# slitvinov/PINN_for_quantum_wavefunction_surfaces

Measured on NVIDIA B200. Metric: collocation points/sec per training step (fwd+lap+bwd), higher is better.
Workload: dtype f32

## Files before the change

### include/pinn_b200.h

```cpp
#ifndef PINN_B200_H
#define PINN_B200_H

#include <stdint.h>

#ifdef __cplusplus
extern "C" {
#endif

#define PINN_THETA_SIZE 1521
#define PINN_NUM_TENSORS 16
#define PINN_SUMS_SIZE 8

#define PINN_VARIANT_POC 0
#define PINN_VARIANT_TRAINPY 1

#define PINN_F32 0
#define PINN_F64 1

#define PINN_EINVAL (-1)
#define PINN_ENOTSUP (-2)
#define PINN_ETIMEDOUT (-3)

typedef struct pinn_handle pinn_handle;

int pinn_version(void);
int pinn_theta_size(void);
void pinn_theta_offsets(int* out);

int pinn_create(int device, pinn_handle** out);
int pinn_destroy(pinn_handle* h);
const char* pinn_last_error(pinn_handle* h);
int64_t pinn_launch_count(pinn_handle* h);

#define PINN_ENGINE_FFMA 0
#define PINN_ENGINE_TCGEN05 1
int pinn_set_engine(pinn_handle* h, int engine);
int pinn_get_engine(pinn_handle* h);

int pinn_measure_fp32_peak(pinn_handle* h, double* fma_per_s, double* ms, double* sm_mhz);
int pinn_step_kernel_clock(pinn_handle* h, void* stream, double* cycles, double* ns);

int pinn_host_timing(pinn_handle* h, double* out4);

int pinn_profile_begin(pinn_handle* h);
int pinn_profile_collect(pinn_handle* h, double* total_ms, int* launches);

int pinn_loss_fwd_bwd(pinn_handle* h, int variant, int64_t n,
                      const void* x, const void* y, const void* z, const void* R, int in_dtype,
                      const uint8_t* mask, const float* theta, const double* weights,
                      uint32_t grad_mask, float bcutoff,
                      double* sums, double* dtheta, float* E_out, void* stream);

int pinn_fields(pinn_handle* h, int variant, int64_t n,
                const void* x, const void* y, const void* z, const void* R, int in_dtype,
                const float* theta,
                float* psi, float* lap, float* hpsi, float* res, float* E, void* stream);

int pinn_loss_fwd_bwd_tensors(pinn_handle* h, int variant, int64_t n,
                              const void* x, const void* y, const void* z, const void* R, int in_dtype,
                              const uint8_t* mask, const void* const* params, int param_dtype, int param_layout,
                              const double* weights_host, uint32_t grad_mask, float bcutoff,
                              double* sums, double* dtheta, void* E_out, int E_dtype, void* stream);

int pinn_mask_from_index_sets(pinn_handle* h, int64_t n, const int64_t* idx1, int64_t n1, const int64_t* idx2, int64_t n2,
                              uint8_t* mask, void* stream);

int pinn_loss_fwd_bwd_host(pinn_handle* h, int variant, int64_t n,
                           const void* x, const void* y, const void* z, const void* R, int in_dtype,
                           const uint8_t* mask, const double* theta_host, const double* weights_host,
                           uint32_t grad_mask, float bcutoff,
// ... 61 lines not shown
```

### pinn_for_quantum_wavefunction_surfaces_b200/_lib.py

```python
import ctypes
import os
import threading

_HERE = os.path.dirname(os.path.abspath(__file__))
_LIB_NAME = "libpinn_b200.so"

EXPORTS = [
    "pinn_version", "pinn_theta_size", "pinn_theta_offsets", "pinn_create", "pinn_destroy", "pinn_last_error",
    "pinn_launch_count", "pinn_set_engine", "pinn_get_engine", "pinn_profile_begin", "pinn_profile_collect", "pinn_loss_fwd_bwd", "pinn_fields", "pinn_loss_fwd_bwd_host",
    "pinn_loss_fwd_bwd_tensors", "pinn_mask_from_index_sets", "pinn_measure_fp32_peak", "pinn_step_kernel_clock",
    "pinn_sample", "pinn_adam_step", "pinn_enet_curve", "pinn_grid_reduce", "pinn_spheroidal_reduce", "pinn_trainer_create", "pinn_trainer_destroy",
    "pinn_trainer_load_state", "pinn_trainer_set_batch", "pinn_trainer_run", "pinn_trainer_read", "pinn_trainer_batch",
    "pinn_trainer_stream",
    "pinn_host_timing", "pinn_dp_init", "pinn_dp_connect", "pinn_dp_connect_local", "pinn_dp_enable", "pinn_dp_status", "pinn_dp_set_timeout", "pinn_dp_shutdown",
]


class TrainConfig(ctypes.Structure):
    _fields_ = [("variant", ctypes.c_int), ("best_mode", ctypes.c_int), ("history_mean_E", ctypes.c_int),
                ("sc_sampling", ctypes.c_int), ("n", ctypes.c_int64), ("freeze_after", ctypes.c_int64),
                ("best_after", ctypes.c_int64), ("history_capacity", ctypes.c_int64), ("seed", ctypes.c_uint64),
                ("xL", ctypes.c_float), ("xR", ctypes.c_float), ("yL", ctypes.c_float), ("yR", ctypes.c_float),
                ("zL", ctypes.c_float), ("zR", ctypes.c_float), ("RL", ctypes.c_float), ("RR", ctypes.c_float),
                ("cutoff", ctypes.c_float), ("bcutoff", ctypes.c_float), ("grad_mask", ctypes.c_uint32),
                ("lr", ctypes.c_double), ("beta1", ctypes.c_double), ("beta2", ctypes.c_double), ("eps", ctypes.c_double)]


class PinnError(RuntimeError):
    pass


def library_path():
    return os.environ.get("PINN_B200_LIBRARY") or os.path.join(_HERE, _LIB_NAME)


_lib = None
_lock = threading.Lock()


def lib():
    global _lib
    with _lock:
        if _lib is not None:
            return _lib
        path = library_path()
        if not os.path.exists(path):
            raise PinnError("%s not found: build it with `python -c 'import __graft_entry__ as g; g.build()'` "
                            "(there is no CPU fallback)" % path)
        L = ctypes.CDLL(path)
        vp, i32, i64, u32, f32 = ctypes.c_void_p, ctypes.c_int, ctypes.c_int64, ctypes.c_uint32, ctypes.c_float
        L.pinn_version.restype = i32
        L.pinn_theta_size.restype = i32
        L.pinn_theta_offsets.argtypes = [ctypes.POINTER(i32)]
        L.pinn_theta_offsets.restype = None
        L.pinn_create.argtypes = [i32, ctypes.POINTER(vp)]
        L.pinn_create.restype = i32
        L.pinn_destroy.argtypes = [vp]
        L.pinn_destroy.restype = i32
        L.pinn_last_error.argtypes = [vp]
        L.pinn_last_error.restype = ctypes.c_char_p
        L.pinn_launch_count.argtypes = [vp]
        L.pinn_launch_count.restype = i64
        L.pinn_set_engine.argtypes = [vp, i32]
        L.pinn_set_engine.restype = i32
        L.pinn_get_engine.argtypes = [vp]
        L.pinn_get_engine.restype = i32
        L.pinn_profile_begin.argtypes = [vp]
        L.pinn_profile_begin.restype = i32
        L.pinn_profile_collect.argtypes = [vp, ctypes.POINTER(ctypes.c_double), ctypes.POINTER(i32)]
        L.pinn_profile_collect.restype = i32
        L.pinn_loss_fwd_bwd.argtypes = [vp, i32, i64, vp, vp, vp, vp, i32, vp, vp, vp, u32, f32, vp, vp, vp, vp]
        L.pinn_loss_fwd_bwd.restype = i32
        L.pinn_loss_fwd_bwd_tensors.argtypes = [vp, i32, i64, vp, vp, vp, vp, i32, vp, vp, i32, i32, vp, u32, f32, vp, vp, vp, i32, vp]
        L.pinn_loss_fwd_bwd_tensors.restype = i32
        L.pinn_mask_from_index_sets.argtypes = [vp, i64, vp, i64, vp, i64, vp, vp]
        L.pinn_mask_from_index_sets.restype = i32
        L.pinn_measure_fp32_peak.argtypes = [vp, ctypes.POINTER(ctypes.c_double), ctypes.POINTER(ctypes.c_double),
                                             ctypes.POINTER(ctypes.c_double)]
        L.pinn_measure_fp32_peak.restype = i32
        L.pinn_step_kernel_clock.argtypes = [vp, vp, ctypes.POINTER(ctypes.c_double), ctypes.POINTER(ctypes.c_double)]
        L.pinn_step_kernel_clock.restype = i32
        L.pinn_fields.argtypes = [vp, i32, i64, vp, vp, vp, vp, i32, vp, vp, vp, vp, vp, vp, vp]
        L.pinn_fields.restype = i32
        L.pinn_loss_fwd_bwd_host.argtypes = [vp, i32, i64, vp, vp, vp, vp, i32, vp, vp, vp, u32, f32, vp, vp, vp]
        L.pinn_loss_fwd_bwd_host.restype = i32
        u64, f64 = ctypes.c_uint64, ctypes.c_double
        L.pinn_sample.argtypes = [vp, i64, u64, u64, ctypes.POINTER(f32), f32, f32, vp, vp, vp, vp, vp, vp, vp, vp]
        L.pinn_sample.restype = i32
        L.pinn_adam_step.argtypes = [vp, vp, vp, vp, vp, vp, vp, vp, vp, vp, vp, vp, i64, i64, f64, f64, f64, f64, u32,
                                     i32, i64, i32, vp]
        L.pinn_adam_step.restype = i32
        L.pinn_enet_curve.argtypes = [vp, vp, vp, i32, vp, vp, vp, vp, vp]
        L.pinn_enet_curve.restype = i32
        L.pinn_grid_reduce.argtypes = [vp, i32, vp, i32, i32, i32, ctypes.POINTER(f64), f64, vp, vp, vp, vp, vp]
        L.pinn_grid_reduce.restype = i32
        L.pinn_spheroidal_reduce.argtypes = [vp, i32, vp, i32, vp, i32, vp, vp, i32, vp, vp, vp, vp]
        L.pinn_spheroidal_reduce.restype = i32
        L.pinn_trainer_create.argtypes = [vp, ctypes.POINTER(TrainConfig), vp, ctypes.POINTER(vp)]
        L.pinn_trainer_create.restype = i32
# ... 60 lines not shown
    _cache = {}
    _cache_lock = threading.Lock()

    def __init__(self, device=0):
        self.L = lib()
        self.device = int(device)
        hp = ctypes.c_void_p()
        rc = self.L.pinn_create(self.device, ctypes.byref(hp))
        if rc != 0:
            raise PinnError("pinn_create(device=%d) failed (%d): %s"
                            % (device, rc, self.L.pinn_last_error(None).decode()))
        self.h = hp

    @classmethod
    def get(cls, device=0):
        device = int(device)
        with cls._cache_lock:
            if device not in cls._cache:
                cls._cache[device] = Handle(device)
            return cls._cache[device]

    def check(self, rc, what):
        if rc != 0:
            raise PinnError("%s failed (%d): %s" % (what, rc, self.L.pinn_last_error(self.h).decode()))

    def launch_count(self):
        return int(self.L.pinn_launch_count(self.h))

    ENGINES = {"ffma": 0, "tcgen05": 1}

    def set_engine(self, name):
        self.check(self.L.pinn_set_engine(self.h, self.ENGINES[name]), "pinn_set_engine")

    def get_engine(self):
        return {v: k for k, v in self.ENGINES.items()}[int(self.L.pinn_get_engine(self.h))]

    def measure_fp32_peak(self):
        r, ms, mhz = ctypes.c_double(), ctypes.c_double(), ctypes.c_double()
        self.check(self.L.pinn_measure_fp32_peak(self.h, ctypes.byref(r), ctypes.byref(ms), ctypes.byref(mhz)), "pinn_measure_fp32_peak")
        return 2.0 * r.value, ms.value, mhz.value

    def step_kernel_clock(self, stream):
        c, ns = ctypes.c_double(), ctypes.c_double()
        self.check(self.L.pinn_step_kernel_clock(self.h, ctypes.c_void_p(stream), ctypes.byref(c), ctypes.byref(ns)), "pinn_step_kernel_clock")
        return c.value / ns.value * 1e3 if ns.value > 0 else 0.0

    def profile_begin(self):
        self.check(self.L.pinn_profile_begin(self.h), "pinn_profile_begin")

    def profile_collect(self):
        ms, k = ctypes.c_double(), ctypes.c_int()
        self.check(self.L.pinn_profile_collect(self.h, ctypes.byref(ms), ctypes.byref(k)), "pinn_profile_collect")
        return ms.value, k.value

    DP_HANDLE_BYTES = 64

    def dp_init(self, rank, world, want_ipc=True):
        buf = ctypes.create_string_buffer(self.DP_HANDLE_BYTES)
        self.check(self.L.pinn_dp_init(self.h, int(rank), int(world), buf if want_ipc else None), "pinn_dp_init")
        return bytes(buf.raw)

    def dp_connect(self, all_handles):
        blob = b"".join(all_handles)
        self.check(self.L.pinn_dp_connect(self.h, ctypes.c_char_p(blob)), "pinn_dp_connect")

    def dp_connect_local(self, handles):
# ... 27 lines not shown
```

### pinn_for_quantum_wavefunction_surfaces_b200/csrc/pinn_capi.cu

```cuda
#include <chrono>
#include <cstdio>
#include <cstdlib>
#include <cstring>
#include <mutex>
#include <string>
#include <vector>

#include "pinn_handle.h"
#include "pinn_train.h"

std::string g_create_err;

constexpr int HOST_IN_THETA = 1536;
constexpr size_t HOST_IN_BYTES = HOST_IN_THETA * sizeof(float) + 4 * sizeof(double);

static const int kOffsets[17] = {O_W1, O_B1, O_W2, O_B2, O_WO, O_BO, O_WE1, O_BE1, O_WE2, O_BE2, O_WE, O_BE,
                                 O_WGL, O_BGL, O_WG, O_BG, NTHETA};

extern "C" {

int pinn_version(void) { return 100; }
int pinn_theta_size(void) { return NTHETA; }
void pinn_theta_offsets(int* out) { memcpy(out, kOffsets, sizeof(kOffsets)); }

// ... 24 lines not shown
#ifdef PINN_AB_BUILD
  if (const char* e = getenv("PINN_B200_ENGINE")) {
    if (!strcmp(e, "ffma")) h->engine = PINN_ENGINE_FFMA;
    else if (!strcmp(e, "tcgen05")) h->engine = PINN_ENGINE_TCGEN05;
  }
  if (const char* e = getenv("PINN_B200_HOST_ZEROCOPY")) h->host_zero_copy = strcmp(e, "0") != 0;
  if (const char* e = getenv("PINN_B200_HOST_INLINE")) h->host_inline_params = strcmp(e, "0") != 0;
  CREATE_CU(cudaMalloc(&h->wts, sizeof(Wts)));
#endif
  CREATE_CU(cudaMalloc(&h->theta_dev, HOST_IN_BYTES));
  h->weights_dev = reinterpret_cast<double*>(h->theta_dev + HOST_IN_THETA);
  CREATE_CU(cudaHostAlloc(&h->out_pinned, NPART * sizeof(double), cudaHostAllocMapped));
  CREATE_CU(cudaHostGetDevicePointer(&h->out_mapped, h->out_pinned, 0));
  CREATE_CU(cudaMallocHost(&h->theta_pinned, HOST_IN_BYTES));
  h->weights_pinned = reinterpret_cast<double*>(h->theta_pinned + HOST_IN_THETA);
  CREATE_CU(cudaStreamCreateWithFlags(&h->s_copy, cudaStreamNonBlocking));
  CREATE_CU(cudaStreamCreateWithFlags(&h->s_main, cudaStreamNonBlocking));
  CREATE_CU(cudaEventCreateWithFlags(&h->ev_copy, cudaEventDisableTiming));
  for (int c = 0; c < 4; c++) CREATE_CU(cudaEventCreateWithFlags(&h->ev_chunk[c], cudaEventDisableTiming));
  if (!ws_for(h, h->s_main, 4 * h->sm_count)) {
    const std::string msg = h->err;
    pinn_destroy(h);
    g_create_err = "pinn_create: " + msg;
    return PINN_EINVAL;
  }
  *out = h;
  return 0;
}

}

static void ws_free(pinn_workspace& w) {
  cudaFree(w.partials); cudaFree(w.weights); cudaFree(w.counts); cudaFree(w.grid_partials); cudaFree(w.sph_partials);
  w = pinn_workspace();
}

void ws_release(pinn_handle* h, cudaStream_t st) {
  for (pinn_workspace& c : h->ws)
    if (c.stream == st && c.partials) {
      cudaStreamSynchronize(st);
      ws_free(c);
    }
}

static bool stream_is_capturing(cudaStream_t st) {
  cudaStreamCaptureStatus cap = cudaStreamCaptureStatusNone;
  if (cudaStreamIsCapturing(st, &cap) != cudaSuccess) { cudaGetLastError(); return false; }
  return cap != cudaStreamCaptureStatusNone;
}

pinn_workspace* ws_for(pinn_handle* h, cudaStream_t st, int rows) {
  constexpr size_t MAX_WS = 32;
  pinn_workspace* w = nullptr;
  for (pinn_workspace& c : h->ws)
    if (c.stream == st && c.partials) { w = &c; break; }
  if (w && w->rows >= rows) {
    if (!w->in_graph && stream_is_capturing(st)) w->in_graph = true;
    w->last_use = ++h->ws_clock;
    return w;
  }
  if (stream_is_capturing(st)) {
    fail(h, PINN_EINVAL, "first call on a stream under CUDA-graph capture: call once on this stream outside the capture first");
    return nullptr;
  }
  if (!w) {
    for (pinn_workspace& c : h->ws)
      if (!c.partials) { w = &c; break; }
    if (!w && h->ws.size() >= MAX_WS) {
      size_t lru = h->ws.size();
      for (size_t i = 0; i < h->ws.size(); i++)
        if (!h->ws[i].in_graph && h->ws[i].stream != h->s_main && (lru == h->ws.size() || h->ws[i].last_use < h->ws[lru].last_use)) lru = i;
      if (lru == h->ws.size()) {
        fail(h, PINN_EINVAL, "more than 32 streams with captured graphs or trainers on one handle");
        return nullptr;
      }
      cudaDeviceSynchronize();
      ws_free(h->ws[lru]);
      w = &h->ws[lru];
    } else if (!w) {
      h->ws.emplace_back();
      w = &h->ws.back();
    }
  } else {
    if (w->in_graph) {
      fail(h, PINN_EINVAL, "this stream's workspace is referenced by a captured graph and cannot grow");
      return nullptr;
    }
    cudaStreamSynchronize(st);
    ws_free(*w);
  }
  w->stream = st;
  cudaError_t e = cudaMalloc(&w->partials, (size_t)rows * NPART * sizeof(double));
  if (e == cudaSuccess) e = cudaMalloc(&w->weights, 4 * sizeof(double));
  if (e == cudaSuccess) e = cudaMalloc(&w->counts, 4 * sizeof(unsigned long long));
  if (e == cudaSuccess) e = cudaMemset(w->counts, 0, 4 * sizeof(unsigned long long));
  if (e == cudaSuccess) e = cudaMalloc(&w->grid_partials, (size_t)(h->sm_count + 1) * 8 * sizeof(double));
  if (e != cudaSuccess) {
    ws_free(*w);
    fail(h, (int)e, "workspace allocation (cudaMalloc)");
    return nullptr;
  }
  w->rows = rows;
  w->last_use = ++h->ws_clock;
  return w;
}

bool ws_sph_rows(pinn_handle* h, pinn_workspace* w, cudaStream_t st, int rows) {
  if (w->sph_rows >= rows) return true;
  if (stream_is_capturing(st)) {
    fail(h, PINN_EINVAL, "spheroidal sweep larger than any earlier one on a stream under CUDA-graph capture: make the largest "
                         "call once on this stream outside the capture first");
    return false;
  }
  if (w->in_graph) {
    fail(h, PINN_EINVAL, "this stream's workspace is referenced by a captured graph and cannot grow");
    return false;
  }
  cudaStreamSynchronize(st);
  cudaFree(w->sph_partials);
  w->sph_partials = nullptr;
  w->sph_rows = 0;
  cudaError_t e = cudaMalloc(&w->sph_partials, (size_t)rows * 8 * sizeof(double));
  if (e != cudaSuccess) {
    w->sph_partials = nullptr;
    fail(h, (int)e, "spheroidal workspace allocation (cudaMalloc)");
    return false;
  }
  w->sph_rows = rows;
  return true;
// ... 33 lines not shown
  DevGuard dev_guard(h->device);
  dp_release(h);
  cudaDeviceSynchronize();
#ifdef PINN_AB_BUILD
  cudaFree(h->wts);
#endif
  for (pinn_workspace& w : h->ws) ws_free(w);
  cudaFree(h->theta_dev); cudaFree(h->stage_dev);
  cudaFreeHost(h->out_pinned); cudaFreeHost(h->theta_pinned);
  if (h->s_copy) cudaStreamDestroy(h->s_copy);
  if (h->s_main) cudaStreamDestroy(h->s_main);
  if (h->ev_copy) cudaEventDestroy(h->ev_copy);
  for (int c = 0; c < 4; c++) if (h->ev_chunk[c]) cudaEventDestroy(h->ev_chunk[c]);
  for (cudaEvent_t e : h->ev_pool) cudaEventDestroy(e);
  delete h;
  return 0;
}

const char* pinn_last_error(pinn_handle* h) { return h ? h->err.c_str() : g_create_err.c_str(); }
int64_t pinn_launch_count(pinn_handle* h) { return h ? h->launches : 0; }

int pinn_set_engine(pinn_handle* h, int engine) {
  if (!h) return PINN_EINVAL;
  std::lock_guard<std::mutex> lk(h->mu);
  if (engine != PINN_ENGINE_FFMA && engine != PINN_ENGINE_TCGEN05) return fail(h, PINN_EINVAL, "pinn_set_engine: unknown engine");
#ifndef PINN_AB_BUILD
  if (engine != PINN_ENGINE_TCGEN05)
    return fail(h, PINN_ENOTSUP, "pinn_set_engine: this library carries the tcgen05 engine only (the FFMA engine exists in A/B builds, tools/build_ab.sh)");
#endif
  h->engine = engine;
  return 0;
}
int pinn_get_engine(pinn_handle* h) { return h ? h->engine : PINN_EINVAL; }

int pinn_host_timing(pinn_handle* h, double* out4) {
  if (!h || !out4) return PINN_EINVAL;
  memcpy(out4, h->host_us, sizeof(h->host_us));
  return 0;
}

int pinn_profile_begin(pinn_handle* h) {
  if (!h) return PINN_EINVAL;
  std::lock_guard<std::mutex> lk(h->mu);
  h->profiling = true;
  h->ev_used = 0;
  return 0;
}

int pinn_profile_collect(pinn_handle* h, double* total_ms, int* launches) {
  if (!h || !total_ms || !launches) return PINN_EINVAL;
  std::lock_guard<std::mutex> lk(h->mu);
  DevGuard dev_guard(h->device);
  double tot = 0.0;
  for (size_t i = 0; i + 1 < h->ev_used; i += 2) {
    CU(h, cudaEventSynchronize(h->ev_pool[i + 1]));
    float ms = 0.0f;
    CU(h, cudaEventElapsedTime(&ms, h->ev_pool[i], h->ev_pool[i + 1]));
    tot += ms;
  }
  *total_ms = tot;
  *launches = (int)(h->ev_used / 2);
  h->profiling = false;
  h->ev_used = 0;
  return 0;
}

// ... 184 lines not shown
    return fail(h, PINN_EINVAL, "pinn_loss_fwd_bwd: NULL pointer argument");
  if (c.in_dtype != PINN_F32 && c.in_dtype != PINN_F64) return fail(h, PINN_EINVAL, "pinn_loss_fwd_bwd: bad in_dtype");
  DevGuard dev_guard(h->device);
  pinn_workspace* ws = ws_for(h, st, h->sm_count);
  if (!ws) return PINN_EINVAL;
  if (int rc = dp_serialize(h, st)) return rc;
  p.x = c.x; p.y = c.y; p.z = c.z; p.R = c.R; p.mask = c.mask; p.n = c.n; p.in_f64 = c.in_dtype == PINN_F64;
  p.bcut = c.bcutoff; p.partials = ws->partials; p.E_out = static_cast<float*>(c.E_out); p.E_f64 = c.E_f64;
  p.base_grads = (c.grad_mask & 0x003Fu) != 0;
  p.gate_grads = (c.grad_mask & 0xF000u) != 0;
  const double* weights = c.weights;
  if (c.theta_inline) {
    p.theta_inline = c.theta_inline;
  } else if (c.theta_tensors) {
#ifdef PINN_AB_BUILD
    if (h->engine != PINN_ENGINE_TCGEN05) return fail(h, PINN_ENOTSUP, "the FFMA engine takes a packed theta only");
#endif
    for (int k = 0; k < 16; k++) {
      if (!c.theta_tensors[k]) return fail(h, PINN_EINVAL, "pinn_loss_fwd_bwd_tensors: NULL parameter tensor");
      p.theta_tensors[k] = c.theta_tensors[k];
    }
    p.theta_from_tensors = 1; p.tensors_f64 = c.tensors_f64; p.tensors_in_out = c.tensors_in_out;
  } else {
    if (int rc = enqueue_prep(h, c.theta, p, st)) return rc;
  }
  if (c.weights_inline) {
    p.weights_inline = c.weights_inline;
  } else if (!weights) {
    CU(h, launch_count(p, ws->counts, ws->weights, st));
    h->launches += 2;
    weights = ws->weights;
  }
  p.weights = weights;
  int grid = 0;
  int rc = enqueue_step_chunk(h, ws, nev, p, 0, c.n, 0, &grid, st);
  if (rc) return rc;
  CU(h, launch_reduce(ws->partials, grid, weights, c.weights_inline, c.grad_mask, c.dtheta, c.sums, p.E_out, c.n,
                      h->dp_on ? h->dp : DpArgs(), st, c.adam, c.adam_ticket, c.presample, c.E_f64, c.dtheta_in_out));
  h->launches++;
  return 0;
}

extern "C" {

int pinn_loss_fwd_bwd(pinn_handle* h, int variant, int64_t n, const void* x, const void* y, const void* z,
                      const void* R, int in_dtype, const uint8_t* mask, const float* theta, const double* weights,
                      uint32_t grad_mask, float bcutoff, double* sums, double* dtheta, float* E_out, void* stream) {
  if (!h) return PINN_EINVAL;
  if (!theta) return fail(h, PINN_EINVAL, "pinn_loss_fwd_bwd: NULL pointer argument");
  LossCall c;
  c.variant = variant; c.n = n; c.x = x; c.y = y; c.z = z; c.R = R; c.in_dtype = in_dtype; c.mask = mask;
  c.theta = theta; c.weights = weights; c.grad_mask = grad_mask; c.bcutoff = bcutoff; c.sums = sums; c.dtheta = dtheta;
  c.E_out = E_out;
  return loss_fwd_bwd_impl(h, c, (cudaStream_t)stream);
}

int pinn_loss_fwd_bwd_tensors(pinn_handle* h, int variant, int64_t n, const void* x, const void* y, const void* z,
                              const void* R, int in_dtype, const uint8_t* mask, const void* const* params, int param_dtype,
                              int param_layout, const double* weights_host, uint32_t grad_mask, float bcutoff, double* sums,
                              double* dtheta, void* E_out, int E_dtype, void* stream) {
  if (!h) return PINN_EINVAL;
  if (!params) return fail(h, PINN_EINVAL, "pinn_loss_fwd_bwd_tensors: NULL pointer argument");
  if ((param_dtype != PINN_F32 && param_dtype != PINN_F64) || (E_dtype != PINN_F32 && E_dtype != PINN_F64) ||
      (param_layout != PINN_VARIANT_POC && param_layout != PINN_VARIANT_TRAINPY))
    return fail(h, PINN_EINVAL, "pinn_loss_fwd_bwd_tensors: bad dtype / layout code");
  static const int kTrainpyToCanonical[16] = {0, 1, 2, 3, 4, 5, 12, 13, 14, 15, 6, 7, 8, 9, 10, 11};
  const void* canon[16];
  for (int k = 0; k < 16; k++) canon[param_layout == PINN_VARIANT_TRAINPY ? kTrainpyToCanonical[k] : k] = params[k];
  LossCall c;
// ... 171 lines not shown
```

### pinn_for_quantum_wavefunction_surfaces_b200/csrc/pinn_device.cuh

```cuda
#pragma once
#include "pinn_common.cuh"
#include "pinn_launch.h"

namespace pinn {

constexpr int ROWH = 64;
constexpr int ROWE = 32;
constexpr int EVAL_STASH = 2 * 32 * ROWH;
constexpr int ENET_STASH = 2 * 32 * ROWE;

__device__ __forceinline__ int swz(int row) { return (row & 3) << 3; }
__host__ __device__ constexpr int swz_tc(int row) { return ((((row & 3) << 1) | ((row >> 2) & 1)) << 2); }

__device__ __forceinline__ float rcp_approx(float x) {
  float r;
  asm("rcp.approx.ftz.f32 %0, %1;" : "=f"(r) : "f"(x));
  return r;
}
__device__ __forceinline__ float sigm(float u) {
  float e;
  asm("ex2.approx.ftz.f32 %0, %1;" : "=f"(e) : "f"(u * -1.4426950408889634f));
  return rcp_approx(1.0f + e);
}

// ... 207 lines not shown
  };
  for (int i = t; i < NH * NH; i += nt) {
    const int j = i / NH, k = i % NH;
    const float wjk = th[O_W2 + i];
    const float a = th[O_W1 + 2 * k], b = th[O_W1 + 2 * k + 1];
    put(out->BS[0], out->BS[1], umma_off(j, k, NH), wjk);
    put(out->BSP[0], out->BSP[1], umma_off(j, k, 2 * NH), wjk * a);
    put(out->BSP[0], out->BSP[1], umma_off(NH + j, k, 2 * NH), wjk * b);
    put(out->BSPP[0], out->BSPP[1], umma_off(j, k, 3 * NH), wjk * (a * a));
    put(out->BSPP[0], out->BSPP[1], umma_off(NH + j, k, 3 * NH), wjk * (a * b));
    put(out->BSPP[0], out->BSPP[1], umma_off(2 * NH + j, k, 3 * NH), wjk * (b * b));
    put(out->BWT[0], out->BWT[1], umma_off(k, j, NH), wjk);
  }
  for (int i = t; i < NE * NE; i += nt) {
    const int j = i / NE, k = i % NE;
    put(out->BE[0], out->BE[1], umma_off(j, k, NE), th[O_WE2 + i]);
    put(out->BET[0], out->BET[1], umma_off(k, j, NE), th[O_WE2 + i]);
  }
}

__device__ __forceinline__ void st_relaxed_sys_v2(unsigned int* p, unsigned int a, unsigned int b) {
  asm volatile("st.relaxed.sys.global.v2.u32 [%0], {%1, %2};" ::"l"(p), "r"(a), "r"(b) : "memory");
}
__device__ __forceinline__ uint2 ld_relaxed_sys_v2(const unsigned int* p) {
  uint2 v;
  asm volatile("ld.relaxed.sys.global.v2.u32 {%0, %1}, [%2];" : "=r"(v.x), "=r"(v.y) : "l"(p) : "memory");
  return v;
}
__device__ __forceinline__ double ld_acquire_gpu(const double* p) {
  double v;
  asm volatile("ld.acquire.gpu.global.f64 %0, [%1];" : "=d"(v) : "l"(p) : "memory");
  return v;
}
__device__ __forceinline__ void st_release_sys(unsigned long long* p, unsigned long long v) {
  asm volatile("st.release.sys.global.u64 [%0], %1;" ::"l"(p), "l"(v) : "memory");
}
__device__ __forceinline__ unsigned long long ld_acquire_sys(const unsigned long long* p) {
  unsigned long long v;
  asm volatile("ld.acquire.sys.global.u64 %0, [%1];" : "=l"(v) : "l"(p) : "memory");
  return v;
}

__device__ __forceinline__ float2 sigm2_pre(const float2 up) {
  const float2 d = __fadd2_rn(make_float2(ex2_approx(up.x), ex2_approx(up.y)), make_float2(1.0f, 1.0f));
  return make_float2(rcp_approx(d.x), rcp_approx(d.y));
}

__device__ __forceinline__ float2 one_minus_sigm2(const float2 e, const float2 s) {
  return make_float2(__saturatef(__fmul_rn(e.x, s.x)), __saturatef(__fmul_rn(e.y, s.y)));
}

__device__ __forceinline__ float2 sigm2_pre(const float2 up, float2& om) {
  const float2 e = make_float2(ex2_approx(up.x), ex2_approx(up.y));
  const float2 d = __fadd2_rn(e, make_float2(1.0f, 1.0f));
  const float2 s = make_float2(rcp_approx(d.x), rcp_approx(d.y));
  om = one_minus_sigm2(e, s);
  return s;
}

__device__ __forceinline__ float2 one_minus_sigm2_pre(const float2 up, const float2 s) {
  return one_minus_sigm2(make_float2(ex2_approx(up.x), ex2_approx(up.y)), s);
}

__device__ __forceinline__ float sigm_pre(float up) { return rcp_approx(1.0f + ex2_approx(up)); }

__device__ __forceinline__ float2 quad_form2(float al11, float al12, float al22, float2 v1, float2 v2) {
// ... 8 lines not shown
```

### pinn_for_quantum_wavefunction_surfaces_b200/csrc/pinn_handle.h

```cpp
#pragma once
#include <cstdio>
#include <mutex>
#include <string>
#include <vector>

#include "../../include/pinn_b200.h"
#include "pinn_common.cuh"
#include "pinn_launch.h"

using namespace pinn;

struct pinn_workspace {
  cudaStream_t stream = nullptr;
  double* partials = nullptr;
  int rows = 0;
  double* weights = nullptr;
  unsigned long long* counts = nullptr;
  double* grid_partials = nullptr;
  double* sph_partials = nullptr;
  int sph_rows = 0;
  uint64_t last_use = 0;
  bool in_graph = false;
};

struct pinn_handle {
  int device = 0;
  int sm_count = 0;
  std::vector<pinn_workspace> ws;
  uint64_t ws_clock = 0;
#ifdef PINN_AB_BUILD
  Wts* wts = nullptr;
#endif
  float* theta_dev = nullptr;
  double* weights_dev = nullptr;
  void* stage_dev = nullptr;
  size_t stage_bytes = 0;
  double* out_pinned = nullptr;
  double* out_mapped = nullptr;
  float* theta_pinned = nullptr;
  double* weights_pinned = nullptr;
  cudaStream_t s_copy = nullptr, s_main = nullptr;
  cudaEvent_t ev_copy = nullptr;
  cudaEvent_t ev_chunk[4] = {nullptr, nullptr, nullptr, nullptr};
  unsigned char* dp_buf = nullptr;
  DpArgs dp;
  bool dp_on = false;
  cudaStream_t dp_stream = nullptr;
  bool dp_stream_set = false;
  bool dp_opened[DP_MAX_WORLD] = {false, false, false, false, false, false, false, false};
  double host_us[4] = {0, 0, 0, 0};
  int64_t launches = 0;
  int engine = PINN_ENGINE_TCGEN05;
  bool host_inline_params = true;
  bool host_zero_copy = true;
  bool profiling = false;
  std::vector<cudaEvent_t> ev_pool;
  size_t ev_used = 0;
  std::string err;
  std::mutex mu;
  std::mutex host_mu;
};

struct DevGuard {
  int prev = -1, dev;
  explicit DevGuard(int d) : dev(d) {
    if (cudaGetDevice(&prev) != cudaSuccess) prev = -1;
    if (prev != dev) cudaSetDevice(dev);
  }
  ~DevGuard() {
    if (prev >= 0 && prev != dev) cudaSetDevice(prev);
  }
  DevGuard(const DevGuard&) = delete;
  DevGuard& operator=(const DevGuard&) = delete;
};

namespace pinn { struct AdamParams; struct SampleParams; }
struct LossCall {
  int variant = 0;
  int64_t n = 0;
  const void *x = nullptr, *y = nullptr, *z = nullptr, *R = nullptr;
  int in_dtype = PINN_F32;
  const uint8_t* mask = nullptr;
  const float* theta = nullptr;
  const float* theta_inline = nullptr;
  const void* const* theta_tensors = nullptr;
  int tensors_f64 = 0, tensors_in_out = 0;
  const double* weights = nullptr;
// ... 36 lines not shown
```

### pinn_for_quantum_wavefunction_surfaces_b200/csrc/pinn_launch.h

```cpp
#pragma once
#include <cstdint>
#include <cuda_runtime.h>

#include "pinn_common.cuh"

namespace pinn {

struct GridDesc {
  int on;
  int sph;
  int nx, ny, nz;
  double x0, dx, y0, dy, z0, dz;
  double R;
  const double *wx, *wy, *wz;
  double* partials;
  int ns, nnu, tiles_per_R;
  const double *Rs, *s, *ws, *nu, *wnu;
};

struct StepParams {
  const void *x, *y, *z, *R;
  const uint8_t* mask;
  const Wts* wts;
  const float* theta;
  const double* weights;
  double* partials;
  float* E_out;
  float *psi, *lap, *hpsi, *res;
  long long n;
  int in_f64;
  float bcut;
  VariantCoef vc;
  int base_grads, gate_grads;
  GridDesc grid;
  const float* theta_inline;
  const double* weights_inline;
  int w_by_value;
  const void* theta_tensors[16];
  int theta_from_tensors, tensors_f64, tensors_in_out;
  int E_f64;
};

template <typename... KArgs, typename... Args>
inline cudaError_t launch_pdl(void (*kernel)(KArgs...), dim3 grid, dim3 block, size_t smem, cudaStream_t st, Args&&... args) {
  cudaLaunchConfig_t cfg = {};
  cfg.gridDim = grid;
  cfg.blockDim = block;
  cfg.dynamicSmemBytes = smem;
  cfg.stream = st;
  cudaLaunchAttribute attr[1];
  attr[0].id = cudaLaunchAttributeProgrammaticStreamSerialization;
  attr[0].val.programmaticStreamSerializationAllowed = 1;
  cfg.attrs = attr;
  cfg.numAttrs = 1;
  return cudaLaunchKernelEx(&cfg, kernel, static_cast<KArgs>(args)...);
}
#ifdef __CUDACC__
__device__ __forceinline__ void pdl_wait() { asm volatile("griddepcontrol.wait;" ::: "memory"); }
__device__ __forceinline__ void pdl_launch_dependents() { asm volatile("griddepcontrol.launch_dependents;" ::: "memory"); }
#endif

#ifdef PINN_AB_BUILD
cudaError_t launch_step(int nev, bool train, const StepParams& p, int grid, cudaStream_t st);
cudaError_t launch_prep(const float* theta, Wts* out, cudaStream_t st);
#endif
cudaError_t launch_step_tc(int nev, bool train, const StepParams& p, int grid, cudaStream_t st);
cudaError_t launch_grid_finish(const double* partials, int nrows, double* out, cudaStream_t st);
cudaError_t launch_sph_finish(const double* partials, int nR, int rows_per_R, const double* Rs, double* out, cudaStream_t st);
cudaError_t launch_count(const StepParams& p, unsigned long long* counts, double* weights, cudaStream_t st);
constexpr int DP_MAX_WORLD = 8;
constexpr long long DP_TIMEOUT_CYCLES = 60000000000ll;
constexpr int DP_BLOCKS = NPART / 32;
constexpr size_t DP_ROWS_BYTES = 2ull * DP_MAX_WORLD * NPART * 16;
// ... 20 lines not shown
```

### pinn_for_quantum_wavefunction_surfaces_b200/csrc/pinn_reduce.cu

```cuda
#include "pinn_device.cuh"
#include "pinn_sample.cuh"
#include "pinn_train.h"

namespace pinn {


__global__ void count_sets_kernel(const StepParams p, unsigned long long* counts) {
  unsigned c1 = 0, c2 = 0;
  for (long long i = (long long)blockIdx.x * blockDim.x + threadIdx.x; i < p.n; i += (long long)gridDim.x * blockDim.x) {
    if (p.mask) {
      const unsigned mk = p.mask[i];
      c1 += mk & 1u; c2 += (mk >> 1) & 1u;
    } else {
      const Geom g = load_geom(p, i);
      c1 += (g.ir1 * p.bcut <= 1.0f); c2 += (g.ir2 * p.bcut <= 1.0f);
    }
  }
  c1 = __reduce_add_sync(0xffffffffu, c1);
  c2 = __reduce_add_sync(0xffffffffu, c2);
  if ((threadIdx.x & 31) == 0) { atomicAdd(&counts[0], c1); atomicAdd(&counts[1], c2); }
}
__global__ void weights_from_counts_kernel(const unsigned long long* counts, long long n, double* w) {
  w[0] = 1.0 / (double)n;
  w[1] = 1.0 / (double)counts[0];
// ... 71 lines not shown
        const long long t0 = clock64();
        uint2 lo = make_uint2(0u, 0u), hi = lo;
        bool ok = false;
        while (!dp_failed_s) {
          lo = ld_relaxed_sys_v2(src);
          hi = ld_relaxed_sys_v2(src + 2);
          if (lo.y == step && hi.y == step) { ok = true; break; }
          if (clock64() - t0 > dp.timeout_cycles) {
            for (int q = 0; q < dp.world; q++)
              st_release_sys(reinterpret_cast<unsigned long long*>(dp.peer[q] + DP_ROWS_BYTES) + 2, 1ull);
            dp_failed_s = 1;
            break;
          }
        }
        v = ok ? __longlong_as_double((long long)(((unsigned long long)hi.x << 32) | lo.x)) : 0.0;
      }
    }
    __syncthreads();
    sh[sl][e] = v;
    __syncthreads();
    if (threadIdx.x == 0) {
      __threadfence();
      if (atomicAdd(&ctl[1], 1ull) == (unsigned long long)DP_BLOCKS - 1) {
        ctl[1] = 0ull;
        st_release_sys(&ctl[0], step64);
      }
    }
  }
  if (sl == 0) {
    double t = 0.0;
#pragma unroll
    for (int i = 0; i < RED_SLICES; i++) t += sh[i][e];
    tot[e] = t;
    if (idx < NTHETA) {
      int ti, off;
      theta_locate(idx, ti, off);
      const int dst = dtheta_in_out ? off + in_out_index(ti, idx - off) : idx;
      dtheta[dst] = ((grad_mask >> ti) & 1u) ? t : 0.0;
    }
  }
  __syncthreads();
  const double w0 = wi.use ? wi.w[0] : weights[0], w1 = wi.use ? wi.w[1] : weights[1], w2 = wi.use ? wi.w[2] : weights[2];
  constexpr int SB = S_RES2 / 32, b = S_RES2 - SB * 32;
  if (blockIdx.x == SB && threadIdx.x == 0) {
    const double r2 = tot[b], p1 = tot[b + 1], p2 = tot[b + 2], sE = tot[b + 3];
    const double Lpde = w0 * r2, Lbc = w1 * p1 + w2 * p2;
    sums[0] = Lpde + Lbc; sums[1] = Lpde; sums[2] = Lbc; sums[3] = sE;
    sums[4] = r2; sums[5] = p1; sums[6] = p2;
    sums[7] = (E_out && n > 0) ? (E_f64 ? reinterpret_cast<const double*>(E_out)[n - 1] : (double)E_out[n - 1]) : 0.0;
  }
  if (!ad.on) return;

  if (blockIdx.x == SB) {
    if (threadIdx.x < 3) l3[threadIdx.x] = tot[b + threadIdx.x];
  } else {
    if (threadIdx.x < 96) {
      const int j = threadIdx.x >> 5, sj = threadIdx.x & 31;
      double ps = 0.0;
#pragma unroll 5
      for (int r = sj; r < nrows; r += RED_SLICES) ps += partials[(size_t)r * NPART + S_RES2 + j];
      sh[sj][j] = ps;
    }
    __syncthreads();
    if (threadIdx.x < 3) {
      const int j = threadIdx.x;
      double local = 0.0;
#pragma unroll
      for (int i = 0; i < RED_SLICES; i++) local += sh[i][j];
      double g = local;
      if (dp.world > 1) {
        const unsigned char* own = dp.peer[dp.rank];
        g = 0.0;
        for (int r = 0; r < dp.world; r++) {
          double v = local;
          if (r != dp.rank) {
            const unsigned int* src = reinterpret_cast<const unsigned int*>(own) + ((slot + r) * NPART + S_RES2 + j) * 4;
            const long long t0 = clock64();
            uint2 lo = make_uint2(0u, 0u), hi = lo;
            bool ok = false;
            while (!dp_failed_s) {
              lo = ld_relaxed_sys_v2(src);
              hi = ld_relaxed_sys_v2(src + 2);
              if (lo.y == step && hi.y == step) { ok = true; break; }
// ... 88 lines not shown
```

### pinn_for_quantum_wavefunction_surfaces_b200/csrc/pinn_step_tc.cu

```cuda
#include <cstring>
#include <type_traits>

#include "pinn_tc.cuh"

#ifdef PINN_TIMELINE
__device__ long long g_timeline[16 * 32];
#define TL(i) do { if (blockIdx.x == 0 && c.tl_it == 3 && (threadIdx.x & 31) == 0) g_timeline[(threadIdx.x >> 5) * 32 + (i)] = clock64(); } while (0)
extern "C" int pinn_debug_timeline(long long* out) { return (int)cudaMemcpyFromSymbol(out, g_timeline, sizeof(g_timeline)); }
__device__ long long g_timeline_k[48];
__device__ long long g_timeline_cta[2 * 256];
extern "C" int pinn_debug_timeline_cta(long long* out) { return (int)cudaMemcpyFromSymbol(out, g_timeline_cta, sizeof(g_timeline_cta)); }
#define TLK(i) do { if (blockIdx.x == 0 && threadIdx.x == 0) g_timeline_k[(i)] = clock64(); \
                    if (threadIdx.x == 0 && ((i) == 0 || (i) == 41)) { unsigned long long t_; asm volatile("mov.u64 %0, %%globaltimer;" : "=l"(t_)); \
                      g_timeline_cta[blockIdx.x * 2 + ((i) == 41)] = (long long)t_; } } while (0)
extern "C" int pinn_debug_timeline_kernel(long long* out) { return (int)cudaMemcpyFromSymbol(out, g_timeline_k, sizeof(g_timeline_k)); }
#else
#define TL(i) do { } while (0)
#define TLK(i) do { } while (0)
#endif

namespace pinn {


template <int NEV>
// ... 580 lines not shown
      float2 om;
      const float2 s2 = sigm2_pre(f2fma(f2bc(R), make_float2(w.WgLs[i], w.WgLs[i + 1]), make_float2(w.bgLs[i], w.bgLs[i + 1])), om);
      const float2 ub = gate_grads ? f2mul(f2mul(f2bc(gbar), make_float2(w.wg[i], w.wg[i + 1])), f2mul(om, s2)) : f2bc(0.0f);
      const float2 ur = f2mul(ub, f2bc(R));
      const float2 gs = gate_grads ? f2mul(f2bc(gbar), s2) : f2bc(0.0f);
      ch[i] = ur.x; ch[i + 1] = ur.y;
      ch[10 + i] = ub.x; ch[10 + i + 1] = ub.y;
      ch[20 + i] = gs.x; ch[20 + i + 1] = gs.y;
    }
    ch[30] = gate_grads ? gbar : 0.0f;
    ch[31] = Ebar;
#pragma unroll
    for (int c4 = 0; c4 < 32; c4 += 4) ST4(&E1row[c4 ^ sx], ch[c4], ch[c4 + 1], ch[c4 + 2], ch[c4 + 3]);
  }
  __syncwarp();
  {
    float2 plain, weighted;
    colsum2_w<ROWE>(Vs, 2 * (lane & 15), lane >> 4, R, plain, weighted);
    acc2(acc.s2, weighted);
    acc2(acc.s3, plain);
  }
  acc2(acc.s4, colsum2<ROWE>(E1s, 2 * (lane & 15), lane >> 4));
  __syncwarp();
}

template <typename EntryOf>
__device__ __forceinline__ void fold_pair(float* __restrict__ myrow, float2 v, int lane, EntryOf entry_of) {
  v.x += __shfl_xor_sync(0xffffffffu, v.x, 16);
  v.y += __shfl_xor_sync(0xffffffffu, v.y, 16);
  if (lane < 16) {
    const int a = entry_of(2 * lane), b = entry_of(2 * lane + 1);
    if (a >= 0) myrow[a] = v.x;
    if (b >= 0) myrow[b] = v.y;
  }
}

constexpr int TC_REG_MLP = 184, TC_REG_ENET = 136;
static_assert(128 * TC_REG_ENET + 256 * TC_REG_MLP <= 384 * 168, "register rebalancing must fit the launch allocation");

struct TcParamsPlain {
  StepParams p;
  double w[4];
};
struct TcParamsInline {
  StepParams p;
  double w[4];
  alignas(16) float theta[NTHETA + 3];
};

template <int NEV, bool TRAIN, bool INLINE>
__global__ void __launch_bounds__((NEV + 1) * 128, 1)
pinn_step_tc_kernel(const __grid_constant__ typename std::conditional<INLINE, TcParamsInline, TcParamsPlain>::type q) {
  const StepParams& p = q.p;
  constexpr int G = 4;
  extern __shared__ __align__(128) unsigned char smem_raw[];
  Wts& w = *reinterpret_cast<Wts*>(smem_raw);
  uint64_t* mbars = reinterpret_cast<uint64_t*>(smem_raw + WTS_TC_BYTES);
  uint32_t* tmem_slot = reinterpret_cast<uint32_t*>(smem_raw + WTS_TC_BYTES + 32);
  uint64_t* cfull = reinterpret_cast<uint64_t*>(smem_raw + WTS_TC_BYTES + 40);
  float2* mbox = reinterpret_cast<float2*>(smem_raw + WTS_TC_BYTES + 64);
  float* stash = reinterpret_cast<float*>(smem_raw + WTS_TC_BYTES + 64 + sizeof(float2) * G * 2 * 3 * 32);
  unsigned char* cstage = smem_raw + tc_smem_bytes<NEV>() - COORD_STAGES * COORD_STAGE_BYTES - GEO_BYTES;
  float4* geo = reinterpret_cast<float4*>(smem_raw + tc_smem_bytes<NEV>() - GEO_BYTES);

  const int tid = threadIdx.x, lane = tid & 31;
  const int warp = __shfl_sync(0xffffffffu, tid >> 5, 0);
// ... 385 lines not shown
        for (int mt = 0; mt < 2; mt++)
  #pragma unroll
          for (int nt = 0; nt < 4; nt++) {
            const int j0 = mt * 16 + gq, j1 = j0 + 8, k0 = nt * 8 + 2 * tq, k1 = k0 + 1;
            myrow[O_WE2 + j0 * NE + k0] = acc.c[mt][nt][0];
            myrow[O_WE2 + j0 * NE + k1] = acc.c[mt][nt][1];
            myrow[O_WE2 + j1 * NE + k0] = acc.c[mt][nt][2];
            myrow[O_WE2 + j1 * NE + k1] = acc.c[mt][nt][3];
          }
        fold_pair(myrow, acc.s0, lane, [](int i) { return (int)O_WE + i; });
        fold_pair(myrow, acc.s1, lane, [](int i) { return (int)O_BE2 + i; });
        fold_pair(myrow, acc.s2, lane, [](int i) { return (int)O_WE1 + i; });
        fold_pair(myrow, acc.s3, lane, [](int i) { return (int)O_BE1 + i; });
        fold_pair(myrow, acc.s4, lane, [](int i) {
          return i < 10 ? (int)O_WGL + i : i < 20 ? (int)O_BGL + i - 10 : i < 30 ? (int)O_WG + i - 20 : i == 30 ? (int)O_BG : (int)O_BE;
        });
      }
    }
    __syncthreads();
    constexpr int nwarps = (NEV + 1) * G;
    double* row = p.partials + (size_t)blockIdx.x * NPART;
    for (int i = tid; i < NPART; i += blockDim.x) {
      int w0, w1;
      if (i < O_BO) { w0 = 0; w1 = NEV * G; }
      else if (i == O_BO || (i >= S_RES2 && i <= S_CNT2)) { w0 = 0; w1 = G; }
      else if (i < NTHETA) { w0 = NEV * G; w1 = nwarps; }
      else { w0 = 0; w1 = 0; }
      double sum = 0.0;
      for (int wv = w0; wv < w1; wv++) sum += (double)stash[wv * NPART + i];
      if (i >= NPART - 2 && blockIdx.x == 0) sum = reinterpret_cast<const double*>(mbox)[i - (NPART - 2)];
      row[i] = sum;
    }
    TLK(41);
  };
  constexpr bool REBALANCE = TRAIN && NEV == 2;
  if (is_mlp) {
    if constexpr (REBALANCE) asm volatile("setmaxnreg.inc.sync.aligned.u32 %0;" ::"n"(TC_REG_MLP));
    run_role(std::true_type{});
  } else {
    if constexpr (REBALANCE) asm volatile("setmaxnreg.dec.sync.aligned.u32 %0;" ::"n"(TC_REG_ENET));
    run_role(std::false_type{});
  }
}

template <int NEV, bool TRAIN, bool INLINE>
static cudaError_t launch_step_tc_t(const StepParams& p, int grid, cudaStream_t st) {
  auto kern = pinn_step_tc_kernel<NEV, TRAIN, INLINE>;
  constexpr size_t smem = tc_smem_bytes<NEV>();
  static bool configured[16] = {false};
  int dev = 0;
  cudaGetDevice(&dev);
  if (dev < 16 && !configured[dev]) {
    cudaError_t e = cudaFuncSetAttribute(kern, cudaFuncAttributeMaxDynamicSharedMemorySize, (int)smem);
    if (e != cudaSuccess) return e;
    configured[dev] = true;
  }
  if constexpr (INLINE) {
    TcParamsInline q;
    q.p = p;
    memcpy(q.theta, p.theta_inline, NTHETA * sizeof(float));
    q.theta[NTHETA] = q.theta[NTHETA + 1] = q.theta[NTHETA + 2] = 0.0f;
    q.w[0] = q.w[1] = q.w[2] = q.w[3] = 0.0;
    if (p.weights_inline) memcpy(q.w, p.weights_inline, 3 * sizeof(double));
    q.p.w_by_value = p.weights_inline != nullptr;
    return launch_pdl(kern, dim3(grid), dim3((NEV + 1) * 128), smem, st, q);
  } else {
// ... 56 lines not shown
```

Baseline: 2.318 billion.

## Fuse final gradient reduction into step kernel via last-block tickets

Adds an in-kernel finish path. Blocks take atomic tickets, the last block of each of 32 classes sums that class's partial rows, and the last class block sums the class rows and writes dtheta and the loss sums directly. This removes the separate reduce kernel launch and its dependency gap when data-parallel exchange, Adam and presampling are off. In exchange, the tail of the step kernel is serialized on a few blocks and adds threadfences and atomics.

```diff
diff --git a/include/pinn_b200.h b/include/pinn_b200.h
--- a/include/pinn_b200.h
+++ b/include/pinn_b200.h
@@ -36,6 +36,8 @@
 #define PINN_ENGINE_TCGEN05 1
 int pinn_set_engine(pinn_handle* h, int engine);
 int pinn_get_engine(pinn_handle* h);
+
+int pinn_set_step_finish(pinn_handle* h, int on);
 
 int pinn_measure_fp32_peak(pinn_handle* h, double* fma_per_s, double* ms, double* sm_mhz);
 int pinn_step_kernel_clock(pinn_handle* h, void* stream, double* cycles, double* ns);
diff --git a/pinn_for_quantum_wavefunction_surfaces_b200/_lib.py b/pinn_for_quantum_wavefunction_surfaces_b200/_lib.py
--- a/pinn_for_quantum_wavefunction_surfaces_b200/_lib.py
+++ b/pinn_for_quantum_wavefunction_surfaces_b200/_lib.py
@@ -7,7 +7,7 @@
 
 EXPORTS = [
     "pinn_version", "pinn_theta_size", "pinn_theta_offsets", "pinn_create", "pinn_destroy", "pinn_last_error",
-    "pinn_launch_count", "pinn_set_engine", "pinn_get_engine", "pinn_profile_begin", "pinn_profile_collect", "pinn_loss_fwd_bwd", "pinn_fields", "pinn_loss_fwd_bwd_host",
+    "pinn_launch_count", "pinn_set_engine", "pinn_get_engine", "pinn_set_step_finish", "pinn_profile_begin", "pinn_profile_collect", "pinn_loss_fwd_bwd", "pinn_fields", "pinn_loss_fwd_bwd_host",
     "pinn_loss_fwd_bwd_tensors", "pinn_mask_from_index_sets", "pinn_measure_fp32_peak", "pinn_step_kernel_clock",
     "pinn_sample", "pinn_adam_step", "pinn_enet_curve", "pinn_grid_reduce", "pinn_spheroidal_reduce", "pinn_trainer_create", "pinn_trainer_destroy",
     "pinn_trainer_load_state", "pinn_trainer_set_batch", "pinn_trainer_run", "pinn_trainer_read", "pinn_trainer_batch",
@@ -65,6 +65,8 @@
         L.pinn_set_engine.restype = i32
         L.pinn_get_engine.argtypes = [vp]
         L.pinn_get_engine.restype = i32
+        L.pinn_set_step_finish.argtypes = [vp, i32]
+        L.pinn_set_step_finish.restype = i32
         L.pinn_profile_begin.argtypes = [vp]
         L.pinn_profile_begin.restype = i32
         L.pinn_profile_collect.argtypes = [vp, ctypes.POINTER(ctypes.c_double), ctypes.POINTER(i32)]
@@ -191,6 +193,9 @@
     def set_engine(self, name):
         self.check(self.L.pinn_set_engine(self.h, self.ENGINES[name]), "pinn_set_engine")
 
+    def set_step_finish(self, on):
+        self.check(self.L.pinn_set_step_finish(self.h, int(bool(on))), "pinn_set_step_finish")
+
     def get_engine(self):
         return {v: k for k, v in self.ENGINES.items()}[int(self.L.pinn_get_engine(self.h))]
 
diff --git a/pinn_for_quantum_wavefunction_surfaces_b200/csrc/pinn_capi.cu b/pinn_for_quantum_wavefunction_surfaces_b200/csrc/pinn_capi.cu
--- a/pinn_for_quantum_wavefunction_surfaces_b200/csrc/pinn_capi.cu
+++ b/pinn_for_quantum_wavefunction_surfaces_b200/csrc/pinn_capi.cu
@@ -80,6 +80,7 @@
 
 static void ws_free(pinn_workspace& w) {
   cudaFree(w.partials); cudaFree(w.weights); cudaFree(w.counts); cudaFree(w.grid_partials); cudaFree(w.sph_partials);
+  cudaFree(w.fin_tickets); cudaFree(w.fin_rows);
   w = pinn_workspace();
 }
 
@@ -143,6 +144,9 @@
   if (e == cudaSuccess) e = cudaMalloc(&w->counts, 4 * sizeof(unsigned long long));
   if (e == cudaSuccess) e = cudaMemset(w->counts, 0, 4 * sizeof(unsigned long long));
   if (e == cudaSuccess) e = cudaMalloc(&w->grid_partials, (size_t)(h->sm_count + 1) * 8 * sizeof(double));
+  if (e == cudaSuccess) e = cudaMalloc(&w->fin_tickets, (FIN_CLASSES + 1) * sizeof(unsigned int));
+  if (e == cudaSuccess) e = cudaMemset(w->fin_tickets, 0, (FIN_CLASSES + 1) * sizeof(unsigned int));
+  if (e == cudaSuccess) e = cudaMalloc(&w->fin_rows, (size_t)FIN_CLASSES * NPART * sizeof(double));
   if (e != cudaSuccess) {
     ws_free(*w);
     fail(h, (int)e, "workspace allocation (cudaMalloc)");
@@ -242,6 +246,13 @@
   return 0;
 }
 int pinn_get_engine(pinn_handle* h) { return h ? h->engine : PINN_EINVAL; }
+
+int pinn_set_step_finish(pinn_handle* h, int on) {
+  if (!h) return PINN_EINVAL;
+  std::lock_guard<std::mutex> lk(h->mu);
+  h->step_finish = on != 0;
+  return 0;
+}
 
 int pinn_host_timing(pinn_handle* h, double* out4) {
   if (!h || !out4) return PINN_EINVAL;
@@ -492,9 +503,16 @@
     weights = ws->weights;
   }
   p.weights = weights;
+  const bool exchange = h->dp_on && h->dp.world > 1;
+  const bool finish = h->step_finish && h->engine == PINN_ENGINE_TCGEN05 && !exchange && !c.adam && !c.presample;
+  if (finish) {
+    p.fin.tickets = ws->fin_tickets; p.fin.class_rows = ws->fin_rows;
+    p.fin.dtheta = c.dtheta; p.fin.sums = c.sums; p.fin.grad_mask = c.grad_mask; p.fin.dtheta_in_out = c.dtheta_in_out;
+  }
   int grid = 0;
   int rc = enqueue_step_chunk(h, ws, nev, p, 0, c.n, 0, &grid, st);
   if (rc) return rc;
+  if (finish) return 0;
   CU(h, launch_reduce(ws->partials, grid, weights, c.weights_inline, c.grad_mask, c.dtheta, c.sums, p.E_out, c.n,
                       h->dp_on ? h->dp : DpArgs(), st, c.adam, c.adam_ticket, c.presample, c.E_f64, c.dtheta_in_out));
   h->launches++;
diff --git a/pinn_for_quantum_wavefunction_surfaces_b200/csrc/pinn_device.cuh b/pinn_for_quantum_wavefunction_surfaces_b200/csrc/pinn_device.cuh
--- a/pinn_for_quantum_wavefunction_surfaces_b200/csrc/pinn_device.cuh
+++ b/pinn_for_quantum_wavefunction_surfaces_b200/csrc/pinn_device.cuh
@@ -263,6 +263,18 @@
   asm volatile("ld.acquire.gpu.global.f64 %0, [%1];" : "=d"(v) : "l"(p) : "memory");
   return v;
 }
+__device__ __forceinline__ void store_dtheta_entry(double* dtheta, int idx, double t, uint32_t grad_mask, int dtheta_in_out) {
+  int ti, off;
+  theta_locate(idx, ti, off);
+  const int dst = dtheta_in_out ? off + in_out_index(ti, idx - off) : idx;
+  dtheta[dst] = ((grad_mask >> ti) & 1u) ? t : 0.0;
+}
+__device__ __forceinline__ void store_loss_sums(double* sums, double r2, double p1, double p2, double sE, double w0, double w1,
+                                                double w2, double E_last) {
+  const double Lpde = w0 * r2, Lbc = w1 * p1 + w2 * p2;
+  sums[0] = Lpde + Lbc; sums[1] = Lpde; sums[2] = Lbc; sums[3] = sE;
+  sums[4] = r2; sums[5] = p1; sums[6] = p2; sums[7] = E_last;
+}
 __device__ __forceinline__ void st_release_sys(unsigned long long* p, unsigned long long v) {
   asm volatile("st.release.sys.global.u64 [%0], %1;" ::"l"(p), "l"(v) : "memory");
 }
diff --git a/pinn_for_quantum_wavefunction_surfaces_b200/csrc/pinn_handle.h b/pinn_for_quantum_wavefunction_surfaces_b200/csrc/pinn_handle.h
--- a/pinn_for_quantum_wavefunction_surfaces_b200/csrc/pinn_handle.h
+++ b/pinn_for_quantum_wavefunction_surfaces_b200/csrc/pinn_handle.h
@@ -17,6 +17,8 @@
   double* weights = nullptr;
   unsigned long long* counts = nullptr;
   double* grid_partials = nullptr;
+  unsigned int* fin_tickets = nullptr;
+  double* fin_rows = nullptr;
   double* sph_partials = nullptr;
   int sph_rows = 0;
   uint64_t last_use = 0;
@@ -53,6 +55,7 @@
   int engine = PINN_ENGINE_TCGEN05;
   bool host_inline_params = true;
   bool host_zero_copy = true;
+  bool step_finish = true;
   bool profiling = false;
   std::vector<cudaEvent_t> ev_pool;
   size_t ev_used = 0;
diff --git a/pinn_for_quantum_wavefunction_surfaces_b200/csrc/pinn_launch.h b/pinn_for_quantum_wavefunction_surfaces_b200/csrc/pinn_launch.h
--- a/pinn_for_quantum_wavefunction_surfaces_b200/csrc/pinn_launch.h
+++ b/pinn_for_quantum_wavefunction_surfaces_b200/csrc/pinn_launch.h
@@ -16,6 +16,16 @@
   double* partials;
   int ns, nnu, tiles_per_R;
   const double *Rs, *s, *ws, *nu, *wnu;
+};
+
+constexpr int FIN_CLASSES = 32;
+struct StepFinish {
+  unsigned int* tickets;
+  double* class_rows;
+  double* dtheta;
+  double* sums;
+  uint32_t grad_mask;
+  int dtheta_in_out;
 };
 
 struct StepParams {
@@ -39,6 +49,7 @@
   const void* theta_tensors[16];
   int theta_from_tensors, tensors_f64, tensors_in_out;
   int E_f64;
+  StepFinish fin;
 };
 
 template <typename... KArgs, typename... Args>
diff --git a/pinn_for_quantum_wavefunction_surfaces_b200/csrc/pinn_reduce.cu b/pinn_for_quantum_wavefunction_surfaces_b200/csrc/pinn_reduce.cu
--- a/pinn_for_quantum_wavefunction_surfaces_b200/csrc/pinn_reduce.cu
+++ b/pinn_for_quantum_wavefunction_surfaces_b200/csrc/pinn_reduce.cu
@@ -127,23 +127,14 @@
 #pragma unroll
     for (int i = 0; i < RED_SLICES; i++) t += sh[i][e];
     tot[e] = t;
-    if (idx < NTHETA) {
-      int ti, off;
-      theta_locate(idx, ti, off);
-      const int dst = dtheta_in_out ? off + in_out_index(ti, idx - off) : idx;
-      dtheta[dst] = ((grad_mask >> ti) & 1u) ? t : 0.0;
-    }
+    if (idx < NTHETA) store_dtheta_entry(dtheta, idx, t, grad_mask, dtheta_in_out);
   }
   __syncthreads();
   const double w0 = wi.use ? wi.w[0] : weights[0], w1 = wi.use ? wi.w[1] : weights[1], w2 = wi.use ? wi.w[2] : weights[2];
   constexpr int SB = S_RES2 / 32, b = S_RES2 - SB * 32;
-  if (blockIdx.x == SB && threadIdx.x == 0) {
-    const double r2 = tot[b], p1 = tot[b + 1], p2 = tot[b + 2], sE = tot[b + 3];
-    const double Lpde = w0 * r2, Lbc = w1 * p1 + w2 * p2;
-    sums[0] = Lpde + Lbc; sums[1] = Lpde; sums[2] = Lbc; sums[3] = sE;
-    sums[4] = r2; sums[5] = p1; sums[6] = p2;
-    sums[7] = (E_out && n > 0) ? (E_f64 ? reinterpret_cast<const double*>(E_out)[n - 1] : (double)E_out[n - 1]) : 0.0;
-  }
+  if (blockIdx.x == SB && threadIdx.x == 0)
+    store_loss_sums(sums, tot[b], tot[b + 1], tot[b + 2], tot[b + 3], w0, w1, w2,
+                    (E_out && n > 0) ? (E_f64 ? reinterpret_cast<const double*>(E_out)[n - 1] : (double)E_out[n - 1]) : 0.0);
   if (!ad.on) return;
 
   if (blockIdx.x == SB) {
diff --git a/pinn_for_quantum_wavefunction_surfaces_b200/csrc/pinn_step_tc.cu b/pinn_for_quantum_wavefunction_surfaces_b200/csrc/pinn_step_tc.cu
--- a/pinn_for_quantum_wavefunction_surfaces_b200/csrc/pinn_step_tc.cu
+++ b/pinn_for_quantum_wavefunction_surfaces_b200/csrc/pinn_step_tc.cu
@@ -636,6 +636,88 @@
     const int a = entry_of(2 * lane), b = entry_of(2 * lane + 1);
     if (a >= 0) myrow[a] = v.x;
     if (b >= 0) myrow[b] = v.y;
+  }
+}
+
+constexpr int FIN_PAIRS = (S_E + 2) / 2;
+template <int NT>
+__device__ __forceinline__ void finish_step(const StepFinish& f, const StepParams& p, const double* w, float* stash, int tid) {
+  constexpr int PPT = (FIN_PAIRS + NT - 1) / NT;
+  constexpr int ROW2 = NPART / 2;
+  volatile int* flag = reinterpret_cast<volatile int*>(stash);
+  double2* tot = reinterpret_cast<double2*>(stash) + 1;
+  const int nb = gridDim.x, cls = blockIdx.x % FIN_CLASSES;
+  const int ncls = nb < FIN_CLASSES ? nb : FIN_CLASSES;
+  __syncthreads();
+  if (tid == 0) {
+    __threadfence();
+    const bool last = atomicAdd(&f.tickets[cls], 1u) == (unsigned)((nb - 1 - cls) / FIN_CLASSES);
+    if (last) __threadfence();
+    flag[0] = last;
+  }
+  __syncthreads();
+  if (!flag[0]) return;
+
+  auto rows_sum = [&](const double2* base, size_t stride, int count, double2 (&acc)[PPT]) {
+    constexpr int B = 8;
+#pragma unroll
+    for (int k = 0; k < PPT; k++) acc[k] = make_double2(0.0, 0.0);
+    for (int j0 = 0; j0 < count; j0 += B) {
+      double2 v[B][PPT];
+#pragma unroll
+      for (int j = 0; j < B; j++)
+#pragma unroll
+        for (int k = 0; k < PPT; k++) {
+          const int i = min(tid + k * NT, FIN_PAIRS - 1);
+          v[j][k] = __ldcg(base + (size_t)min(j0 + j, count - 1) * stride + i);
+        }
+#pragma unroll
+      for (int j = 0; j < B; j++)
+#pragma unroll
+        for (int k = 0; k < PPT; k++) {
+          const double2 x = j0 + j < count ? v[j][k] : make_double2(0.0, 0.0);
+          acc[k].x += x.x; acc[k].y += x.y;
+        }
+    }
+  };
+  {
+    double2 s[PPT];
+    rows_sum(reinterpret_cast<const double2*>(p.partials) + (size_t)cls * ROW2, (size_t)FIN_CLASSES * ROW2,
+             (nb - 1 - cls) / FIN_CLASSES + 1, s);
+    double2* crow = reinterpret_cast<double2*>(f.class_rows) + (size_t)cls * ROW2;
+#pragma unroll
+    for (int k = 0; k < PPT; k++)
+      if (tid + k * NT < FIN_PAIRS) crow[tid + k * NT] = s[k];
+  }
+  __syncthreads();
+  if (tid == 0) {
+    __threadfence();
+    const bool last = atomicAdd(&f.tickets[FIN_CLASSES], 1u) == (unsigned)ncls - 1;
+    if (last) __threadfence();
+    flag[0] = last;
+  }
+  __syncthreads();
+  if (!flag[0]) return;
+
+  double2 t[PPT];
+  rows_sum(reinterpret_cast<const double2*>(f.class_rows), (size_t)ROW2, ncls, t);
+#pragma unroll
+  for (int k = 0; k < PPT; k++) {
+    const int i = tid + k * NT;
+    if (i < FIN_PAIRS) {
+      tot[i] = t[k];
+      if (2 * i < NTHETA) store_dtheta_entry(f.dtheta, 2 * i, t[k].x, f.grad_mask, f.dtheta_in_out);
+      if (2 * i + 1 < NTHETA) store_dtheta_entry(f.dtheta, 2 * i + 1, t[k].y, f.grad_mask, f.dtheta_in_out);
+    }
+  }
+  __syncthreads();
+  if (tid == 0) {
+    const double* td = reinterpret_cast<const double*>(tot);
+    const double E_last = !p.E_out ? 0.0
+                        : p.E_f64 ? __ldcg(reinterpret_cast<const double*>(p.E_out) + (p.n - 1))
+                                  : (double)__ldcg(p.E_out + (p.n - 1));
+    store_loss_sums(f.sums, td[S_RES2], td[S_PSI1], td[S_PSI2], td[S_E], w[0], w[1], w[2], E_last);
+    for (int c = 0; c <= FIN_CLASSES; c++) f.tickets[c] = 0u;
   }
 }
 
@@ -1087,6 +1169,7 @@
       row[i] = sum;
     }
     TLK(41);
+    if (p.fin.tickets) finish_step<(NEV + 1) * 128>(p.fin, p, (INLINE || p.w_by_value) ? q.w : p.weights, stash, tid);
   };
   constexpr bool REBALANCE = TRAIN && NEV == 2;
   if (is_mlp) {
```

After: 2.195 billion (median of 6 runs). 0.947x the previous value.
